# xiph/daala

Measured on NVIDIA H100. Metric: encoder Mpixels/s on 4K YUV420 intra, higher is better.
Workload: dtype int32

## Files before the change

daala_b200/csrc/kf_engine.cu:

```cuda
#include <cuda_runtime.h>
#include <math.h>
#include <stdint.h>
#include <stdio.h>
#include <stdlib.h>
#include <string.h>

#include <algorithm>
#include <cmath>
#include <mutex>
#include <new>
#include <vector>

#include "daala_b200.h"
#include "dering_search.h"
#include "late_skip.h"
#include "lossless.h"
#include "mc_batch.h"
#include "gen/coding_order.inc"
#include "pvq_math.cuh"
#include "pvq_warp.cuh"
#include "pvq_common.cuh"

namespace daala_b200 {
namespace kf {
// ... 628 lines not shown
  int top = -1, left = -1;
  if (band == 0 || r == 1) top = S.dep_top[blk];
  if (band == 0 || r == 2) left = S.dep_left[blk];
  if (band == 3 || band == 6) top = left = -1;
  const int32_t* ot = top >= 0 ? prm.out + prm.blocks[top].coef_off : nullptr;
  const int32_t* ol = left >= 0 ? prm.out + prm.blocks[left].coef_off : nullptr;
  bool low_from_top = false;
  if (band == 0) {
    double g1 = 0, g2 = 0;
    if (ot) { double a = __ldcg(ot + 2), bb = __ldcg(ot + 5), c = __ldcg(ot + 9); g1 += a * a; g1 += bb * bb; g1 += c * c; }
    if (ol) { double a = __ldcg(ol + 1), bb = __ldcg(ol + 4), c = __ldcg(ol + 7); g2 += a * a; g2 += bb * bb; g2 += c * c; }
    low_from_top = g1 > g2;
  }
  int32_t* vref = prm.ref + coef_off;
  for (int i = start + lane; i < start + bn; i += 32) {
    int r2, c2;
    scan_rc(i, &r2, &c2);
    int32_t p = 0;
    if (r2 == 0 && c2 > 0 && ot && (c2 >= 4 || low_from_top)) p = __ldcg(ot + i);
    if (c2 == 0 && r2 > 0 && ol && (r2 >= 4 || !low_from_top)) p = __ldcg(ol + i);
    vref[i] = p;
  }
}

template <bool kIntra>
__device__ __forceinline__ void run_item(const Stage& S, uint32_t item, int lane, int16_t* snap) {
  const daala_b200_pvq_params& prm = S.prm;
  const int blk = (int)(item >> 4), band = (int)(item & 15);
  const daala_b200_pvq_block b = prm.blocks[blk];
  const int bs = b.bs, pli = b.pli;
  const int start = band_start(band);
  const int bn = band_start(band + 1) - start;
  const size_t off = (size_t)b.coef_off + start;
  if (kIntra) intra_band_ref(S, blk, band, b.coef_off, lane);
  int qidx = bs * (bs + 1) + (band + 1) - (band + 1) / 3;
  int q = (prm.q0 * prm.pvq_qm_q4[pli][qidx]) >> 4;
  if (q < 1) q = 1;
  const int beta = (prm.use_masking && pli == 0 && bs > 0) ? kBeta15 : kBeta1;
  const int qoff = (b.xdec & 1 ? prm.qm_stride : 0) + ((((1 << (2 * bs)) - 1) << 4) / 3) + start;
  int itheta, max_theta, k;
  double skip_term;
  const bool pre = kIntra && S.pre_ev && band != 3 && band != 6;
  const int32_t* pev = pre ? S.pre_ev + (off >> 3) * kPreEvWords : nullptr;
  const int16_t* psn = pre ? S.pre_snap + 2 * off : nullptr;
  const int gain = quantise_band_warp<0>(lane, snap, S.rsqrt_tbl, prm.out + off, prm.in + off, prm.ref + off, bn, q,
                                         prm.y + off, &itheta, &max_theta, &k, beta, &skip_term, prm.is_keyframe, pli,
                                         prm.qm + qoff, prm.qm_inv + qoff, prm.pvq_norm_lambda, pev, psn);
  if (lane == 0) {
    const size_t r = (size_t)blk * 9 + band;
    prm.res_skip_term[r] = skip_term;
    short4 pk;
    pk.x = (short)gain; pk.y = (short)itheta; pk.z = (short)max_theta; pk.w = (short)k;
    reinterpret_cast<short4*>(S.res_pack)[r] = pk;
  }
}

struct ItemGeom {
  int blk, band, bn, q, beta, pli, qoff;
  size_t off;
};
__device__ __forceinline__ int band_q(const daala_b200_pvq_params& prm, const daala_b200_kf_frame_quant* fq, int frame,
                                      int pli, int qidx) {
  return fq ? (fq[frame].q0 * fq[frame].pvq_qm_q4[pli][qidx]) >> 4 : (prm.q0 * prm.pvq_qm_q4[pli][qidx]) >> 4;
}
__device__ __forceinline__ ItemGeom item_geom(const daala_b200_pvq_params& prm, uint32_t item,
                                              const daala_b200_kf_frame_quant* fq) {
  ItemGeom g;
  g.blk = (int)(item >> 4);
  g.band = (int)(item & 15);
  const daala_b200_pvq_block b = prm.blocks[g.blk];
  const int bs = b.bs;
  g.pli = b.pli;
  const int start = band_start(g.band);
  g.bn = band_start(g.band + 1) - start;
  g.off = (size_t)b.coef_off + start;
  const int qidx = bs * (bs + 1) + (g.band + 1) - (g.band + 1) / 3;
  int q = band_q(prm, fq, b.frame, g.pli, qidx);
  g.q = q < 1 ? 1 : q;
  g.beta = (prm.use_masking && g.pli == 0 && bs > 0) ? kBeta15 : kBeta1;
  g.qoff = (b.xdec & 1 ? prm.qm_stride : 0) + ((((1 << (2 * bs)) - 1) << 4) / 3) + start;
  return g;
}

template <int kPhase, bool kZeroRef, int kMode, bool kFq = false>
__global__ void __launch_bounds__(128) k_pvq_split(const __grid_constant__ Stage S, int cls, int chunk) {
  const daala_b200_pvq_params& prm = S.prm;
  const int lane = threadIdx.x & 31;
  const int slots = S.sp_slots[cls];
  const int first = chunk * slots;
  const int count = min(S.cnt[S.n_items_at + cls] - first, slots);
  const int vs = cls == 2 ? 128 : 32;
  const int nwarps = (gridDim.x * blockDim.x) >> 5;
  for (int i = (blockIdx.x * blockDim.x + threadIdx.x) >> 5; i < count; i += nwarps) {
    const ItemGeom g = item_geom(prm, S.items[cls][first + i], kFq ? S.fq : nullptr);
    int16_t* vec = S.sp_vec[cls] + (size_t)i * 3 * vs;
    int32_t* lanes = S.sp_lanes[cls] + (size_t)i * kCtxLaneWords * 16;
    int32_t* uni = S.sp_uni[cls] + (size_t)i * kCtxUniWords;
    int16_t* snap = S.sp_snap[cls] + (size_t)i * kMaxEvents * vs;
    const int32_t* r0 = kZeroRef ? nullptr : prm.ref + g.off;
    BandCtx B;
    if (kPhase == 0) {
      band_setup<kMode>(lane, B, prm.in + g.off, r0, g.bn, g.q, g.beta, prm.is_keyframe, g.pli, prm.qm + g.qoff,
                 prm.pvq_norm_lambda, S.rsqrt_tbl);
      band_ctx_store_setup(lane, B, g.bn, vec, vs, lanes, uni);
    } else if (kPhase == 1) {
      band_ctx_load_search(lane, B, g.bn, vec, vs, lanes);
      band_search<kMode>(lane, B, g.bn, snap, vs, S.rsqrt_tbl);
      band_ctx_store_search(lane, B, lanes);
    } else {
      band_ctx_load_finish(lane, B, g.bn, vec, vs, lanes, uni);
      int itheta, max_theta, k;
      double skip_term;
      const int gain = band_finish<kMode>(lane, B, snap, vs, prm.out + g.off, r0, g.bn, g.q, prm.y + g.off, &itheta, &max_theta, &k,
                                   g.beta, &skip_term, prm.is_keyframe, g.pli, prm.qm_inv + g.qoff, prm.pvq_norm_lambda);
      if (lane == 0) {
        const size_t r = (size_t)g.blk * 9 + g.band;
        prm.res_skip_term[r] = skip_term;
        short4 pk;
        pk.x = (short)gain; pk.y = (short)itheta; pk.z = (short)max_theta; pk.w = (short)k;
        reinterpret_cast<short4*>(S.res_pack)[r] = pk;
      }
    }
  }
}

template <int kMode>
__global__ void __launch_bounds__(128) k_pvq_prepass(const __grid_constant__ Stage S) {
  const daala_b200_pvq_params& prm = S.prm;
  __shared__ int16_t snap_all[4][2 * kMaxN];
  const int lane = threadIdx.x & 31;
  int16_t* snap = snap_all[threadIdx.x >> 5];
  const int nblk = min(S.cnt[S.n_blocks_at], S.max_blocks);
  const int nwarps = (gridDim.x * blockDim.x) >> 5;
  const int per = kMode == 2 ? 2 : 5;
  for (long long i = (blockIdx.x * blockDim.x + threadIdx.x) >> 5; i < (long long)nblk * per; i += nwarps) {
    const int blk = (int)(i / per), sel = (int)(i % per);
    const int band = kMode == 2 ? 7 + sel : (sel < 3 ? sel : sel + 1);
    if (band >= num_bands(prm.blocks[blk].bs)) continue;
    const ItemGeom g = item_geom(prm, ((uint32_t)blk << 4) | band, nullptr);
    BandCtx B;
    band_setup<kMode>(lane, B, prm.in + g.off, nullptr, g.bn, g.q, g.beta, prm.is_keyframe, g.pli, prm.qm + g.qoff,
                      prm.pvq_norm_lambda, S.rsqrt_tbl);
    band_search<kMode>(lane, B, g.bn, snap, kMaxN, S.rsqrt_tbl);
    band_noref_export(lane, B, g.bn, snap, kMaxN, S.pre_ev + (g.off >> 3) * kPreEvWords, S.pre_snap + 2 * g.off);
  }
}

__device__ __forceinline__ void grid_barrier(int32_t* bar, int* target, int nctas) {
  __syncthreads();
  if (threadIdx.x == 0) {
    *target += nctas;
    __threadfence();
    atomicAdd(bar, 1);
    while (ld_acquire(bar) < *target) {}
  }
  __syncthreads();
}

__global__ void __launch_bounds__(128, 4) k_pvq_levels(const __grid_constant__ Stage S) {
  const daala_b200_pvq_params& prm = S.prm;
  __shared__ int bar_target;
  if (threadIdx.x == 0) bar_target = 0;
  const int lane = threadIdx.x & 31;
  const int w = (blockIdx.x * blockDim.x + threadIdx.x) >> 5;
  const int nwarps = (gridDim.x * blockDim.x) >> 5;
  const int total = S.cnt[kTotalHi];
  constexpr int vs = 128;
  for (int lvl = 0; lvl < S.nlevels; lvl++) {
    const int base = S.lvl_off[lvl * 3];
    const int end = lvl + 1 < kMaxLevels ? S.lvl_off[(lvl + 1) * 3] : total;
    if (end - base > S.lvl_slots && threadIdx.x == 0 && blockIdx.x == 0) S.cnt[kError] = 2;
    const int n = min(end - base, S.lvl_slots);
    if (n <= 0) continue;
    for (int phase = 0; phase < 3; phase++) {
      for (int i = w; i < n; i += nwarps) {
        const uint32_t item = S.lvl_items[base + i];
        const ItemGeom g = item_geom(prm, item, nullptr);
        int16_t* vec = S.lv_vec + (size_t)i * 3 * vs;
        int32_t* lanes = S.lv_lanes + (size_t)i * kCtxLaneWords * 16;
        int32_t* uni = S.lv_uni + (size_t)i * kCtxUniWords;
        int16_t* snap = S.lv_snap + (size_t)i * kMaxEvents * vs;
        BandCtx B;
        if (phase == 0) {
          intra_band_ref(S, g.blk, g.band, (int)(g.off - band_start(g.band)), lane);
          band_setup<0>(lane, B, prm.in + g.off, prm.ref + g.off, g.bn, g.q, g.beta, prm.is_keyframe, g.pli,
                        prm.qm + g.qoff, prm.pvq_norm_lambda, S.rsqrt_tbl);
          band_ctx_store_setup(lane, B, g.bn, vec, vs, lanes, uni);
        } else if (phase == 1) {
          band_ctx_load_search(lane, B, g.bn, vec, vs, lanes);
          band_search<0>(lane, B, g.bn, snap, vs, S.rsqrt_tbl);
          band_ctx_store_search(lane, B, lanes);
        } else {
          band_ctx_load_finish(lane, B, g.bn, vec, vs, lanes, uni);
          int itheta, max_theta, k;
          double skip_term;
          const int gain = band_finish<0>(lane, B, snap, vs, prm.out + g.off, prm.ref + g.off, g.bn, g.q, prm.y + g.off,
                                          &itheta, &max_theta, &k, g.beta, &skip_term, prm.is_keyframe, g.pli,
                                          prm.qm_inv + g.qoff, prm.pvq_norm_lambda);
          if (lane == 0) {
            const size_t r = (size_t)g.blk * 9 + g.band;
            prm.res_skip_term[r] = skip_term;
            short4 pk;
            pk.x = (short)gain; pk.y = (short)itheta; pk.z = (short)max_theta; pk.w = (short)k;
            reinterpret_cast<short4*>(S.res_pack)[r] = pk;
// ... 507 lines not shown
  }
}

constexpr int kSymSegs = 6;
struct SymCopy {
  const uint8_t* src[kSymSegs];
  uint8_t* dst[kSymSegs];
  long long unit[kSymSegs];
  long long cap[kSymSegs];
  long long index_bytes;
  const long long* tot;
};

__global__ void __launch_bounds__(256) k_sym_copy(const __grid_constant__ SymCopy C) {
  const long long tid = (long long)blockIdx.x * blockDim.x + threadIdx.x;
  const long long nth = (long long)gridDim.x * blockDim.x;
  for (int seg = 0; seg < kSymSegs; seg++) {
    if (!C.dst[seg]) continue;
    const long long want = seg == 0 ? C.index_bytes : C.tot[seg >= 4 ? 0 : seg - 1] * C.unit[seg];
    const long long len = want < C.cap[seg] ? want : C.cap[seg];
    const uint8_t* s = C.src[seg];
    uint8_t* d = C.dst[seg];
    long long done = 0;
    if ((((uintptr_t)s | (uintptr_t)d) & 15) == 0) {
      const long long n16 = len >> 4;
      for (long long i = tid; i < n16; i += nth)
        reinterpret_cast<uint4*>(d)[i] = reinterpret_cast<const uint4*>(s)[i];
      done = n16 << 4;
    }
    for (long long i = done + tid; i < len; i += nth) d[i] = s[i];
  }
}

struct Unstream {
  const uint32_t* order;
  const long long* tot;
  const uint8_t* skip;
  const int32_t* dc;
  uint8_t* fin_skip[2];
  int32_t* fin_dc[2];
  const int32_t* form;
};

__global__ void __launch_bounds__(256) k_fin_unstream(const __grid_constant__ Unstream U) {
  if (!*U.form) return;
  const long long n = U.tot[0];
  for (long long slot = (long long)blockIdx.x * blockDim.x + threadIdx.x; slot < n;
       slot += (long long)gridDim.x * blockDim.x) {
    const uint32_t id = U.order[slot];
    const int ch = id >> 31, blk = (int)(id & 0x7fffffffu);
    U.fin_skip[ch][blk] = U.skip[slot];
    U.fin_dc[ch][blk] = U.dc[slot];
  }
}

}
}

using namespace daala_b200::kf;

extern "C" int daala_b200_launch_forward(const daala_b200_frame* prm, int nplanes, cudaStream_t stream);
extern "C" int daala_b200_launch_inverse(const daala_b200_frame* prm, int nplanes, cudaStream_t stream);
extern "C" int daala_b200_launch_inverse_lapped_only(const daala_b200_frame* prm, int plane0, int nplanes,
                                                     cudaStream_t stream);
extern "C" int daala_b200_launch_sb_postfilter_store(const daala_b200_frame* prm, int plane0, int nplanes,
                                                     cudaStream_t stream);

struct Dering {
  daala_b200_frame frame;
  const uint8_t* skip[3];
  long long skip_pitch[3];
  int skip_stride;
  uint8_t* level;
  const uint8_t* coded;
  uint8_t* applied;
  int tbl[2][6];
  const int32_t* frame_tbl;
  int32_t* thr[2];
  int32_t* dir;
  bool search;
  daala_b200_dering_search_batch sb;
};

enum { kEvLists, kEvForward, kEvLumaBands, kEvLumaScatter, kEvChroma, kNumEvents };

struct daala_b200_kf {
  daala_b200_kf_config cfg;
  int nhsb, nvsb, F;
  int plane_w[3], plane_h[3];
  cudaStream_t stream;
  bool own_stream;
  cudaStream_t side;
  cudaEvent_t ev[kNumEvents];
  cudaGraph_t graph;
  cudaGraphExec_t exec;
  bool captured;
  uint8_t* pixels[3];
  int32_t* coeffs[3];
  int32_t* lapped[3];
  uint8_t* pixels_out[3];
  uint8_t* pred_pixels[3];
  int32_t* pred_coeffs[3];
  uint8_t* bsize;
  int16_t *qm, *qm_inv;
  double* rsqrt_tbl;
  int16_t* sp_vec[3];
  int32_t* sp_lanes[3];
  int32_t* sp_uni[3];
  int16_t* sp_snap[3];
  int sp_slots[3];
  int16_t* lv_vec;
  int32_t* lv_lanes;
  int32_t* lv_uni;
  int16_t* lv_snap;
  int32_t* lv_bar;
  int lvl_slots, lvl_grid;
  Dering dering;
  Lists lists;
  Stage luma, chroma;
  Sym sym;
  daala_b200_frame frame;
  daala_b200_frame frame_pred;
  uint8_t* ref_pixels[3];
  int32_t* ref_slot;
  daala_b200_mv_pt* mv_grid;
  int32_t* ref_slot_next;
  int32_t* mv1_grid;
  uint32_t* mc_leaves;
  int32_t* mc_nleaves;
  daala_b200_mc_batch mc;
  uint8_t* fin_skip[2];
  int32_t* fin_dc[2];
  int32_t* dc_resid[2];
  int32_t* fin_coeffs[3];
  uint8_t* fin_pixels[3];
  uint8_t* fin_bskip[3];
  uint8_t *fin_level, *fin_coded;
  Fin fin;
  cudaGraph_t fin_graph;
  cudaGraphExec_t fin_exec;
  bool fin_captured;
  int fin_dc_limit;
  daala_b200_kf_frame_quant* fq;
  int32_t* fq_tbl;
  std::vector<int32_t> fq_tbl_host;
  int32_t* fin_slot_out;
  PoolStore store;
  uint8_t* fin_stream_skip;
  int32_t* fin_stream_dc;
  int32_t* fin_form;
  Unstream unstream;
  int32_t* d_orig[3];
  daala_b200_kf_late_skip* late_skip[2];
  daala_b200_late_skip_batch lsb;
  int16_t* ll_coeffs[3];
  int32_t* ll_blocks;
  int32_t* ll_dc;
  int32_t* ll_slot_out;
  daala_b200_lossless_batch ll;
  std::vector<uint8_t> slot_filled;
  bool have_step;
  daala_b200_kf_totals last_tot;
  std::vector<void*> allocs;
  size_t bytes_allocated;
  size_t chain_cap;
  int sms;
  char err[256];
// ... 535 lines not shown
      b.nhsb = kf->nhsb;
      b.nvsb = kf->nvsb;
      memcpy(b.threshold, D.tbl[0], sizeof(b.threshold));
      b.coded_quantizer = kf->cfg.coded_quantizer;
      b.qm_is_flat = kf->cfg.qm_is_flat;
      b.use_activity_masking = kf->cfg.use_masking;
      b.dering_lambda = kf->cfg.dering_lambda;
      b.bskip = D.skip[0];
      b.skip_stride = D.skip_stride;
      b.skip_pitch = D.skip_pitch[0];
      b.coded = D.coded;
      b.is_keyframe = inter ? 0 : 1;
      KF_CHECK(dalloc(kf, &b.filt, (size_t)kf->plane_w[0] * kf->plane_h[0] * F));
      KF_CHECK(dalloc(kf, &b.orig, nsb * 4096));
      KF_CHECK(dalloc(kf, &b.cand, nsb * 4096));
      KF_CHECK(dalloc(kf, &b.dist, nsb * 6));
      b.dir = D.dir;
      b.levels = D.level;
      if (kf->cfg.frame_quant) {
        b.fq = kf->fq;
        b.frame_tbl = kf->fq_tbl;
        KF_CHECK(dalloc(kf, &b.cand_thr, nsb * 5));
      }
    }
  }
  KF_CHECK(cudaDeviceSynchronize());
  k_fill_rsqrt<<<(kTableDoubles + 255) / 256, 256, 0, kf->stream>>>(kf->rsqrt_tbl);
  KF_CHECK(cudaGetLastError());
  KF_CHECK(cudaStreamSynchronize(kf->stream));
  return 0;
}

static int enqueue_recon(const daala_b200_frame& frame, int p0, int n, cudaStream_t s) {
  const int rc = daala_b200_launch_inverse_lapped_only(&frame, p0, n, s);
  return rc ? rc : daala_b200_launch_sb_postfilter_store(&frame, p0, n, s);
}

static int enqueue_dering_plane(daala_b200_kf* kf, const Dering& D, int p, cudaStream_t s) {
  const int nsb = kf->nhsb * kf->nvsb;
  const long long per = (long long)kf->plane_w[p] * kf->plane_h[p];
  daala_b200_dering_params dp;
  memset(&dp, 0, sizeof(dp));
  dp.y = nullptr;
  dp.x = D.frame.post16[p];
  dp.dir = D.dir;
  dp.bskip = D.skip[p];
  dp.sb_threshold = D.thr[p ? 1 : 0];
  dp.ystride = dp.xstride = kf->plane_w[p];
  dp.dir_stride = kf->nhsb * 8;
  dp.skip_stride = D.skip_stride;
  dp.nhsb = kf->nhsb;
  dp.nvsb = kf->nvsb;
  dp.xdec = p ? 1 : 0;
  dp.pli = p;
  dp.overlap = 1;
  dp.coeff_shift = 4;
  dp.dir_format = D.search ? 2 : 0;
  return daala_b200_dering_plane_frames(&dp, kf->F, per, per, (long long)nsb * 64, nsb, D.skip_pitch[p],
                                        D.frame.plane[p].pixels_out, s);
}

static int enqueue_dering_luma(daala_b200_kf* kf, const Dering& D, cudaStream_t s) {
  if (D.search) {
    const int rc = daala_b200_dering_search_enqueue(&D.sb, s);
    if (rc) return rc;
  }
  const int nsb = kf->nhsb * kf->nvsb;
  k_dering_thresholds<<<(kf->F * nsb + 255) / 256, 256, 0, s>>>(
      D.level, D.thr[0], D.thr[1], kf->F * nsb, make_int4(D.tbl[0][0], D.tbl[0][1], D.tbl[0][2], D.tbl[0][3]),
      make_int2(D.tbl[0][4], D.tbl[0][5]), make_int4(D.tbl[1][0], D.tbl[1][1], D.tbl[1][2], D.tbl[1][3]),
      make_int2(D.tbl[1][4], D.tbl[1][5]), D.coded, D.applied, D.frame_tbl, nsb);
  return enqueue_dering_plane(kf, D, 0, s);
}

static int enqueue_dering(daala_b200_kf* kf, const Dering& D, cudaStream_t s) {
  int rc = enqueue_recon(D.frame, 0, 3, s);
  if (!rc) rc = enqueue_dering_luma(kf, D, s);
  for (int p = 1; !rc && p < 3; p++) rc = enqueue_dering_plane(kf, D, p, s);
  return rc;
}

static int dering_launches(const Dering& D, int parts) { return 2 * parts + (D.search ? 5 + 6 + 6 + 1 : 0) + 1 + 3; }

template <bool kZeroRef, bool kFq = false>
static void enqueue_split(daala_b200_kf* kf, const Stage& S, cudaStream_t s) {
  const int grid = kf->sms * 16;
  for (int cls = 2; cls >= 0; cls--) {
    for (int chunk = 0; chunk < S.sp_chunks[cls]; chunk++) {
      if (cls == 2) {
        k_pvq_split<0, kZeroRef, 2, kFq><<<grid, 128, 0, s>>>(S, cls, chunk);
        k_pvq_split<1, kZeroRef, 2><<<grid, 128, 0, s>>>(S, cls, chunk);
        k_pvq_split<2, kZeroRef, 2, kFq><<<grid, 128, 0, s>>>(S, cls, chunk);
      } else {
        k_pvq_split<0, kZeroRef, 1, kFq><<<grid, 128, 0, s>>>(S, cls, chunk);
        k_pvq_split<1, kZeroRef, 1><<<grid, 128, 0, s>>>(S, cls, chunk);
        k_pvq_split<2, kZeroRef, 1, kFq><<<grid, 128, 0, s>>>(S, cls, chunk);
      }
    }
  }
}

template <bool kInter>
static void enqueue_sym(const Sym& Y, int wide, cudaStream_t s) {
  k_sym_rank<<<(Y.F * Y.nsb + 7) / 8, 256, 0, s>>>(Y);
  k_sym_sb_scan<<<1, 1024, 0, s>>>(Y);
  k_sym_place<<<wide, 256, 0, s>>>(Y);
  k_sym_tile_sums<<<Y.ntiles, kTile, 0, s>>>(Y);
  k_sym_tile_scan<<<1, 1024, 0, s>>>(Y);
  k_sym_offsets<<<Y.ntiles, kTile, 0, s>>>(Y);
  k_sym_pack<kInter><<<wide, 256, 0, s>>>(Y);
  k_sym_index<<<1, 256, 0, s>>>(Y);
}

static int kf_enqueue_step_inter(daala_b200_kf* kf, int phases) {
  cudaStream_t s = kf->stream;
  const Lists& L = kf->lists;
  const int wide = kf->sms * 8;
  if (phases & DAALA_B200_KF_LISTS) {
    k_unit_tile_sums<<<L.ntiles, kTile, 0, s>>>(L);
    k_tile_scan<<<1, 1024, 0, s>>>(L);
    k_unit_emit<<<L.ntiles, kTile, 0, s>>>(L);
    k_luma_items<<<wide, 256, 0, s>>>(L);
    k_chroma_items<<<wide, 256, 0, s>>>(L);
    if (kf->cfg.inter_mc) {
      if (cudaMemsetAsync(L.cnt + kMcBadRef, 0, 2 * sizeof(int32_t), s) != cudaSuccess) return (int)cudaGetLastError();
      int rc = daala_b200_launch_mc_leaves(&kf->mc, wide, s);
      if (rc) return rc;
    }
  }
  if (phases & DAALA_B200_KF_FORWARD) {
    int rc = kf->cfg.inter_mc ? daala_b200_launch_mc_obmc(&kf->mc, wide, s) : 0;
    if (!rc) rc = daala_b200_launch_forward(&kf->frame, 3, s);
    if (rc) return rc;
    for (int p = 0; kf->cfg.late_skip && p < 3; p++)
      if (cudaMemcpyAsync(kf->d_orig[p], kf->coeffs[p], sizeof(int32_t) * kf->plane_w[p] * kf->plane_h[p] * kf->F,
                          cudaMemcpyDeviceToDevice, s) != cudaSuccess)
        return (int)cudaGetLastError();
    rc = daala_b200_launch_forward(&kf->frame_pred, 3, s);
    if (rc) return rc;
  }
  const bool core = (phases & DAALA_B200_KF_SEARCH_ONLY) != 0;
  for (const Stage* S : {&kf->luma, &kf->chroma}) {
    if (!(phases & (S == &kf->luma ? DAALA_B200_KF_PVQ_LUMA : DAALA_B200_KF_PVQ_CHROMA))) continue;
    if (!core) k_gather<kGatherInter><<<wide, 256, 0, s>>>(*S);
    if (S->fq) enqueue_split<false, true>(kf, *S, s);
    else enqueue_split<false>(kf, *S, s);
    if (!core) k_finish_scatter<true><<<wide, 256, 0, s>>>(*S);
  }
  if (!core && (phases & DAALA_B200_KF_PVQ_CHROMA) && kf->cfg.late_skip) {
    const int rc = daala_b200_late_skip_enqueue(&kf->lsb, kf->sms * 3, s);
    if (rc) return rc;
  }
  if (!core && (phases & DAALA_B200_KF_PVQ_CHROMA) && kf->cfg.symbol_stream) enqueue_sym<true>(kf->sym, wide, s);
  if (phases & DAALA_B200_KF_INVERSE) {
    int rc = daala_b200_launch_inverse(&kf->frame, 3, s);
    if (rc) return rc;
  }
  return (int)cudaGetLastError();
}

static int enqueue_lists(daala_b200_kf* kf, cudaStream_t s) {
  const Lists& L = kf->lists;
  const int wide = kf->sms * 8;
  k_unit_tile_sums<<<L.ntiles, kTile, 0, s>>>(L);
  k_tile_scan<<<1, 1024, 0, s>>>(L);
  k_unit_emit<<<L.ntiles, kTile, 0, s>>>(L);
  const size_t nl = (size_t)L.max_luma * sizeof(int32_t);
  if (cudaMemsetAsync(L.succ_bottom, 0xff, nl, s) != cudaSuccess || cudaMemsetAsync(L.succ_right, 0xff, nl, s) != cudaSuccess)
    return (int)cudaGetLastError();
  if (L.lvl_hist && cudaMemsetAsync(L.lvl_hist, 0, sizeof(int32_t) * kLevelBins, s) != cudaSuccess) return (int)cudaGetLastError();
  if (cudaMemsetAsync(L.head_hist, 0, sizeof(int32_t) * kLevelBins, s) != cudaSuccess) return (int)cudaGetLastError();
  k_luma_deps<<<wide, 256, 0, s>>>(L);
  if (L.lvl_hist) {
    k_level_scan<<<1, 1024, 0, s>>>(L);
    k_level_scatter<<<wide, 256, 0, s>>>(L);
  }
  k_chroma_items<<<wide, 256, 0, s>>>(L);
  return 0;
}

static int enqueue_luma_bands(daala_b200_kf* kf, bool core, int begin, cudaStream_t s) {
  const int wide = kf->sms * 8;
  const int persist = kf->sms * (kf->cfg.persist_ctas_per_sm > 0 ? kf->cfg.persist_ctas_per_sm : kPersistCtas);
  if (cudaMemsetAsync(kf->luma.ring, 0xff, kf->chain_cap * sizeof(uint32_t), s) != cudaSuccess ||
      cudaMemsetAsync(kf->luma.join0, 0, (size_t)kf->luma.max_blocks * sizeof(int32_t), s) != cudaSuccess)
    return (int)cudaGetLastError();
  k_begin_pvq<<<1, 32, 0, s>>>(kf->lists.cnt, begin);
  if (!core) k_gather<kGatherLuma><<<wide, 256, 0, s>>>(kf->luma);
  if (kf->cfg.split_free > 1) enqueue_split<true>(kf, kf->luma, s);
  if (kf->luma.pre_ev) {
    k_pvq_prepass<2><<<kf->sms * 16, 128, 0, s>>>(kf->luma);
    k_pvq_prepass<1><<<kf->sms * 16, 128, 0, s>>>(kf->luma);
  }
  if (kf->cfg.level_chains) {
    if (cudaMemsetAsync(kf->lv_bar, 0, sizeof(int32_t) * 32, s) != cudaSuccess) return (int)cudaGetLastError();
    k_pvq_levels<<<kf->lvl_grid, 128, 0, s>>>(kf->luma);
  } else {
    k_pvq_persist<true><<<persist, kPersistThreads, 0, s>>>(kf->luma);
  }
  return 0;
}

static void enqueue_chroma(daala_b200_kf* kf, bool core, bool begin, cudaStream_t s) {
  const int wide = kf->sms * 8;
  if (begin) k_begin_pvq<<<1, 32, 0, s>>>(kf->lists.cnt, kBeginChroma);
  if (!core) k_gather<kGatherChroma><<<wide, 256, 0, s>>>(kf->chroma);
  if (kf->cfg.split_free > 0) enqueue_split<false>(kf, kf->chroma, s);
  else k_pvq_persist<false><<<kf->sms * (kf->cfg.persist_ctas_per_sm > 0 ? kf->cfg.persist_ctas_per_sm : kPersistCtas),
                              kPersistThreads, 0, s>>>(kf->chroma);
  if (!core) k_finish_scatter<false><<<wide, 256, 0, s>>>(kf->chroma);
}

static int kf_enqueue_step_forked(daala_b200_kf* kf) {
  cudaStream_t s = kf->stream, c = kf->side;
  const daala_b200_frame& fr = kf->cfg.dering ? kf->dering.frame : kf->frame;
  auto fork = [](cudaEvent_t e, cudaStream_t from, cudaStream_t to) {
    return cudaEventRecord(e, from) == cudaSuccess && cudaStreamWaitEvent(to, e, 0) == cudaSuccess;
  };
  if (!fork(kf->ev[kEvLists], s, c)) return (int)cudaGetLastError();
  int rc = daala_b200_launch_forward(&kf->frame, 3, c);
  if (!rc) rc = enqueue_lists(kf, s);
  if (rc) return rc;
  if (!fork(kf->ev[kEvForward], c, s)) return (int)cudaGetLastError();
  rc = enqueue_luma_bands(kf, false, kBeginLuma | kBeginChroma, s);
  if (rc) return rc;
  if (!fork(kf->ev[kEvLumaBands], s, c)) return (int)cudaGetLastError();
  enqueue_chroma(kf, false, false, c);
  k_finish_scatter<false><<<kf->sms * 128, 256, 0, s>>>(kf->luma);
  if (kf->cfg.symbol_stream) {
    if (!fork(kf->ev[kEvLumaScatter], s, c)) return (int)cudaGetLastError();
    enqueue_sym<false>(kf->sym, kf->sms * 8, c);
  }
  rc = enqueue_recon(fr, 1, 2, c);
  if (!rc) rc = enqueue_recon(fr, 0, 1, s);
  if (!rc && kf->cfg.dering) rc = enqueue_dering_luma(kf, kf->dering, s);
  if (rc) return rc;
  if (!fork(kf->ev[kEvChroma], c, s)) return (int)cudaGetLastError();
  for (int p = 1; kf->cfg.dering && p < 3; p++) {
    rc = enqueue_dering_plane(kf, kf->dering, p, s);
    if (rc) return rc;
  }
  return (int)cudaGetLastError();
}

static int kf_enqueue_step_lossless(daala_b200_kf* kf, int phases) {
  if (phases != DAALA_B200_KF_ALL) {
    snprintf(kf->err, sizeof(kf->err), "a lossless step runs whole (DAALA_B200_KF_ALL)");
    return (int)cudaErrorInvalidValue;
  }
  cudaStream_t s = kf->stream;
  const int wide = kf->sms * 8;
  if (kf->cfg.inter_mc) {
    if (cudaMemsetAsync(kf->lists.cnt + kMcBadRef, 0, 2 * sizeof(int32_t), s) != cudaSuccess) return (int)cudaGetLastError();
    int rc = daala_b200_launch_mc_leaves(&kf->mc, wide, s);
    if (!rc) rc = daala_b200_launch_mc_obmc(&kf->mc, wide, s);
    if (rc) return rc;
  }
  return daala_b200_launch_lossless(&kf->ll, s);
}

static int kf_enqueue_step(daala_b200_kf* kf, int phases) {
  if (kf->cfg.lossless) return kf_enqueue_step_lossless(kf, phases);
  if (kf->cfg.inter) return kf_enqueue_step_inter(kf, phases);
  if (phases == DAALA_B200_KF_ALL) return kf_enqueue_step_forked(kf);
  cudaStream_t s = kf->stream;
  if (phases & DAALA_B200_KF_LISTS) {
    const int rc = enqueue_lists(kf, s);
    if (rc) return rc;
  }
  if (phases & DAALA_B200_KF_FORWARD) {
    const int rc = daala_b200_launch_forward(&kf->frame, 3, s);
    if (rc) return rc;
  }
  const bool core = (phases & DAALA_B200_KF_SEARCH_ONLY) != 0;
  if (phases & DAALA_B200_KF_PVQ_LUMA) {
    const int rc = enqueue_luma_bands(kf, core, kBeginLuma, s);
    if (rc) return rc;
    if (!core) k_finish_scatter<false><<<kf->sms * 8, 256, 0, s>>>(kf->luma);
  }
  if (phases & DAALA_B200_KF_PVQ_CHROMA) {
    enqueue_chroma(kf, core, true, s);
    if (!core && kf->cfg.symbol_stream) enqueue_sym<false>(kf->sym, kf->sms * 8, s);
  }
  if (phases & DAALA_B200_KF_INVERSE) {
    int rc = kf->cfg.dering ? enqueue_dering(kf, kf->dering, s) : daala_b200_launch_inverse(&kf->frame, 3, s);
    if (rc) return rc;
  }
  return (int)cudaGetLastError();
}

static int kf_enqueue_finish(daala_b200_kf* kf) {
  cudaStream_t s = kf->stream;
  const int wide = kf->sms * 8;
  if (kf->fin_form) k_fin_unstream<<<wide, 256, 0, s>>>(kf->unstream);
  if (cudaMemsetAsync(kf->fin_coded, 0, (size_t)kf->F * kf->nhsb * kf->nvsb, s) != cudaSuccess)
    return (int)cudaGetLastError();
  k_fin_patch<<<wide, 256, 0, s>>>(kf->fin);
  k_fin_skip_map<<<wide, 256, 0, s>>>(kf->fin);
  const int rc = enqueue_dering(kf, kf->dering, s);
  if (rc) return rc;
  if (kf->fin_slot_out) k_fin_pool_store<<<dim3(wide > kf->F ? wide / kf->F : 1, 3 * kf->F), 256, 0, s>>>(kf->store);
  return (int)cudaGetLastError();
}

extern "C" {

static thread_local char g_create_err[256] = "null engine";

daala_b200_kf* daala_b200_kf_create(const daala_b200_kf_config* cfg) {
  snprintf(g_create_err, sizeof(g_create_err), "daala_b200_kf_create: invalid configuration");
  if (cfg && cfg->inter_mc && (cfg->inter_mc != 1 || cfg->inter != 1)) {
    snprintf(g_create_err, sizeof(g_create_err), "daala_b200_kf_create: inter_mc is 0 or 1, and 1 requires inter = 1");
    return nullptr;
  }
  if (cfg && cfg->mc_next && (cfg->mc_next != 1 || cfg->inter_mc != 1)) {
    snprintf(g_create_err, sizeof(g_create_err), "daala_b200_kf_create: mc_next is 0 or 1, and 1 requires inter_mc = 1");
    return nullptr;
  }
  if (cfg && cfg->inter_finish && (cfg->inter_finish < 0 || cfg->inter_finish > 2 || cfg->inter != 1)) {
    snprintf(g_create_err, sizeof(g_create_err),
             "daala_b200_kf_create: inter_finish is 0, 1 or 2, and 1 and 2 require inter = 1");
    return nullptr;
  }
  if (cfg && (cfg->symbol_stream < 0 || cfg->symbol_stream > 2 || (cfg->symbol_stream == 2 && cfg->inter != 1))) {
    snprintf(g_create_err, sizeof(g_create_err),
             "daala_b200_kf_create: symbol_stream is 0, 1 or 2, and 2 requires inter = 1 (a keyframe's DC goes through "
             "the Haar pyramid and has no scalar index)");
    return nullptr;
  }
  if (cfg && cfg->late_skip && (cfg->late_skip != 1 || cfg->inter != 1)) {
    snprintf(g_create_err, sizeof(g_create_err),
             "daala_b200_kf_create: late_skip is 0 or 1, and 1 requires inter = 1 (keyframes have no late skip)");
    return nullptr;
  }
  if (cfg && cfg->frame_quant && (cfg->frame_quant != 1 || cfg->inter != 1)) {
    snprintf(g_create_err, sizeof(g_create_err),
             "daala_b200_kf_create: frame_quant is 0 or 1, and 1 requires inter = 1 (a keyframe batch shares one quantizer)");
    return nullptr;
  }
  if (cfg && cfg->lossless) {
    const char* with = cfg->lossless != 1 ? "a value other than 0 or 1"
                       : cfg->dering ? "dering (lossless frames skip deringing)"
                       : cfg->symbol_stream ? "symbol_stream (the stream is the PVQ symbols)"
                       : cfg->late_skip ? "late_skip"
                       : cfg->inter_finish ? "inter_finish"
                       : cfg->frame_quant ? "frame_quant (every frame is at quantizer 0)"
                       : cfg->noref_prepass ? "noref_prepass"
                       : cfg->level_chains ? "level_chains"
                       : cfg->sb_rows > 0 ? "a row shard (sb_rows > 0)" : nullptr;
    if (with) {
      snprintf(g_create_err, sizeof(g_create_err), "daala_b200_kf_create: lossless is not defined with %s", with);
      return nullptr;
    }
  }
  if (cfg && cfg->mc_refs < 0) {
    snprintf(g_create_err, sizeof(g_create_err), "daala_b200_kf_create: mc_refs < 0");
    return nullptr;
  }
  if (cfg && cfg->inter) {
    const char* with = cfg->inter != 1 ? "a value other than 0 or 1"
                       : cfg->dering ? "dering (the all-zero skip map of the deringing stage is a keyframe property)"
                       : cfg->symbol_stream == 1 ? "symbol_stream = 1 (its block record has no DC field; "
                                                   "symbol_stream = 2 is the P-frame stream)"
                       : cfg->noref_prepass ? "noref_prepass"
// ... 21 lines not shown
    kf->cfg.sb_row0 = 0;
    kf->cfg.sb_rows = kf->nvsb;
  }
  for (int p = 0; p < 3; p++) {
    kf->plane_w[p] = (kf->nhsb * 64) >> (p ? 1 : 0);
    kf->plane_h[p] = (kf->nvsb * 64) >> (p ? 1 : 0);
  }
  if ((long long)kf->plane_w[0] * kf->plane_h[0] * kf->F >= (1ll << 31)) {
    delete kf;
    return nullptr;
  }
  int dev = 0;
  cudaDeviceProp prop;
  if (cudaGetDevice(&dev) != cudaSuccess || cudaGetDeviceProperties(&prop, dev) != cudaSuccess) {
    delete kf;
    return nullptr;
  }
  kf->sms = prop.multiProcessorCount;
  if (cfg->stream) {
    kf->stream = (cudaStream_t)cfg->stream;
  } else {
    if (cudaStreamCreateWithFlags(&kf->stream, cudaStreamNonBlocking) != cudaSuccess) {
      delete kf;
      return nullptr;
    }
    kf->own_stream = true;
  }
  if (!cfg->inter && !cfg->lossless) {
    int least = 0, greatest = 0;
    bool ok = cudaDeviceGetStreamPriorityRange(&least, &greatest) == cudaSuccess &&
              cudaStreamCreateWithPriority(&kf->side, cudaStreamNonBlocking, greatest) == cudaSuccess;
    for (int i = 0; ok && i < kNumEvents; i++) ok = cudaEventCreateWithFlags(&kf->ev[i], cudaEventDisableTiming) == cudaSuccess;
    if (!ok) {
      snprintf(g_create_err, sizeof(g_create_err), "daala_b200_kf_create: cannot create the second stream and its events");
      daala_b200_kf_destroy(kf);
      return nullptr;
    }
  }
  if (kf_alloc(kf) != 0) {
    fprintf(stderr, "daala_b200_kf_create: %s\n", kf->err);
    snprintf(g_create_err, sizeof(g_create_err), "daala_b200_kf_create: %s", kf->err);
    daala_b200_kf_destroy(kf);
    return nullptr;
  }
  return kf;
}

void daala_b200_kf_destroy(daala_b200_kf* kf) {
  if (!kf) return;
  cudaStreamSynchronize(kf->stream);
  if (kf->exec) cudaGraphExecDestroy(kf->exec);
  if (kf->graph) cudaGraphDestroy(kf->graph);
  if (kf->fin_exec) cudaGraphExecDestroy(kf->fin_exec);
  if (kf->fin_graph) cudaGraphDestroy(kf->fin_graph);
  for (void* p : kf->allocs) cudaFree(p);
  for (cudaEvent_t e : kf->ev)
    if (e) cudaEventDestroy(e);
  if (kf->side) cudaStreamDestroy(kf->side);
  if (kf->own_stream) cudaStreamDestroy(kf->stream);
  delete kf;
}

const char* daala_b200_kf_error(const daala_b200_kf* kf) { return kf ? kf->err : g_create_err; }

#ifdef DAALA_B200_CHAIN_TRACE
int daala_b200_kf_chain_trace(daala_b200_kf* kf, void** recs, int* cap) {
  if (!kf || !recs || !cap) return (int)cudaErrorInvalidValue;
  *recs = kf->luma.trace;
  *cap = kf->luma.trace_cap;
  return 0;
}
#endif

int daala_b200_kf_launches_per_step(const daala_b200_kf* kf) {
  if (!kf) return 0;
  if (kf->cfg.lossless) return (kf->cfg.inter_mc ? 2 : 0) + (kf->cfg.inter ? 1 : 2);
  auto split = [](const Stage& S) { return 3 * (S.sp_chunks[0] + S.sp_chunks[1] + S.sp_chunks[2]); };
  if (kf->cfg.inter)
    return 5 + 2 + (2 + split(kf->luma)) + (2 + split(kf->chroma)) + 2 + (kf->cfg.inter_mc ? 2 : 0) +
           (kf->cfg.symbol_stream ? 8 : 0) + (kf->cfg.late_skip ? kLateSkipLaunches : 0);
  int n = 5 + (kf->cfg.level_chains ? 2 : 0);
  n += 1;
  n += 3 + 1 + (kf->cfg.split_free > 1 ? split(kf->luma) : 0) + (kf->luma.pre_ev ? 2 : 0);
  n += 2 + (kf->cfg.split_free > 0 ? split(kf->chroma) : 1);
  n += kf->cfg.dering ? dering_launches(kf->dering, 2) : 4;
  if (kf->cfg.symbol_stream) n += 8;
  return n;
}

int daala_b200_kf_device_buffers(daala_b200_kf* kf, daala_b200_kf_buffers* out) {
  if (!kf || !out) return (int)cudaErrorInvalidValue;
  memset(out, 0, sizeof(*out));
  for (int p = 0; p < 3; p++) {
    out->pixels[p] = kf->pixels[p];
    out->coeffs[p] = kf->coeffs[p];
    out->lapped[p] = kf->lapped[p];
    out->pixels_out[p] = kf->pixels_out[p];
    out->plane_w[p] = kf->plane_w[p];
    out->plane_h[p] = kf->plane_h[p];
  }
  out->bsize = kf->bsize;
  out->counts = kf->lists.cnt;
  out->luma_blocks = kf->lists.luma;
  out->chroma_blocks = kf->lists.chroma;
  out->dep_top = kf->lists.dep_top;
  out->dep_left = kf->lists.dep_left;
  for (int c = 0; c < 3; c++) {
    out->luma_items[c] = kf->lists.items_l[c];
    out->chroma_items[c] = kf->lists.items_c[c];
  }
  out->luma_heads = kf->lists.heads;
  out->luma_heads0 = kf->lists.heads0;
  out->luma_heads_raw = kf->lists.heads_raw;
  out->luma_head_bin = kf->lists.head_bin;
  out->succ_bottom = kf->lists.succ_bottom;
  out->succ_right = kf->lists.succ_right;
  out->luma_res = kf->luma.res_pack;
  out->chroma_res = kf->chroma.res_pack;
  out->luma_y16 = kf->luma.prm.y16;
  out->chroma_y16 = kf->chroma.prm.y16;
  out->luma_skip_diff = kf->luma.prm.res_skip_diff;
  out->chroma_skip_diff = kf->chroma.prm.res_skip_diff;
  out->chroma_flip = kf->chroma.prm.res_flip;
  out->max_luma_blocks = kf->lists.max_luma;
  out->max_chroma_blocks = kf->lists.max_chroma;
  out->stream = kf->stream;
  out->bytes_allocated = (long long)kf->bytes_allocated;
  for (int p = 0; p < 3; p++) {
    out->pred_pixels[p] = kf->pred_pixels[p];
    out->pred_coeffs[p] = kf->pred_coeffs[p];
    out->ref_pixels[p] = kf->ref_pixels[p];
  }
  out->ref_slot = kf->ref_slot;
  out->mv_grid = kf->mv_grid;
  out->mc_refs = kf->cfg.mc_refs;
  out->ref_slot_next = kf->ref_slot_next;
  out->mv1_grid = kf->mv1_grid;
  out->frame_quant = kf->fq;
  return 0;
}

int daala_b200_kf_run_device(daala_b200_kf* kf, int phases, int use_graph) {
  if (!kf) return (int)cudaErrorInvalidValue;
  if (!use_graph || phases != DAALA_B200_KF_ALL) return kf_enqueue_step(kf, phases);
  if (!kf->captured) {
    int rc = kf_enqueue_step(kf, phases);
    if (rc) return rc;
    KF_CHECK(cudaStreamSynchronize(kf->stream));
    KF_CHECK(cudaStreamBeginCapture(kf->stream, cudaStreamCaptureModeThreadLocal));
    rc = kf_enqueue_step(kf, phases);
    cudaError_t e = cudaStreamEndCapture(kf->stream, &kf->graph);
    if (rc) return rc;
    KF_CHECK(e);
    KF_CHECK(cudaGraphInstantiate(&kf->exec, kf->graph, cudaGraphInstantiateFlagUseNodePriority));
    kf->captured = true;
  }
  KF_CHECK(cudaGraphLaunch(kf->exec, kf->stream));
  return 0;
}

int daala_b200_kf_time_device(daala_b200_kf* kf, int phases, int use_graph, int reps, float* ms) {
  if (!kf || !ms || reps <= 0) return (int)cudaErrorInvalidValue;
  cudaEvent_t e0, e1;
  KF_CHECK(cudaEventCreate(&e0));
  KF_CHECK(cudaEventCreate(&e1));
  if (use_graph && phases == DAALA_B200_KF_ALL && !kf->captured) {
    int rc = daala_b200_kf_run_device(kf, phases, 1);
// ... 482 lines not shown
```

Measured before the change: 2439.

## Fuse chroma CfL gather and scatter into split PVQ phase kernels

When split_free is enabled, the chroma gather and finish-scatter kernels are dropped. Their work moves into phase 0 and phase 2 of the split PVQ kernels, with per-band CfL reference flip, gather and scatter. New k_chroma_records and k_chroma_tail kernels handle per-block bookkeeping and zero the high-frequency tail. The forked schedule is reordered so the chroma tail and records overlap with luma scatter and dering. This is meant to cut separate launches and global round-trips, at the cost of more complex cross-stream ordering and a per-band flip computation that depends on when the DC band is processed.

```diff
diff --git a/daala_b200/csrc/kf_engine.cu b/daala_b200/csrc/kf_engine.cu
--- a/daala_b200/csrc/kf_engine.cu
+++ b/daala_b200/csrc/kf_engine.cu
@@ -734,8 +734,67 @@
   return g;
 }
 
-template <int kPhase, bool kZeroRef, int kMode, bool kFq = false>
-__global__ void __launch_bounds__(128) k_pvq_split(const __grid_constant__ Stage S, int cls, int chunk) {
+constexpr int kFlipScattered = 2;
+
+__device__ __forceinline__ int32_t* block_plane(const daala_b200_pvq_params& prm, const daala_b200_pvq_block& b) {
+  return prm.coef_plane[b.pli] + b.frame * prm.plane_frame_pitch[b.pli] + (size_t)b.y0 * prm.plane_stride[b.pli] + b.x0;
+}
+
+__device__ __forceinline__ void cfl_gather_band(const Stage& S, const ItemGeom& g, int lane) {
+  const daala_b200_pvq_params& prm = S.prm;
+  const daala_b200_pvq_block b = prm.blocks[g.blk];
+  const int ln = b.bs + 2;
+  const int stride = prm.plane_stride[b.pli];
+  const int32_t* src = block_plane(prm, b);
+  const int lo = S.cfl_loff[b.frame * (prm.plane_frame_pitch[b.pli] >> 4) + (long long)(b.y0 >> 2) * (stride >> 2) +
+                            (b.x0 >> 2)];
+  const int rf = g.band ? prm.res_flip[g.blk] : 0;
+  int flip;
+  if (rf & kFlipScattered) {
+    flip = rf & 1;
+  } else {
+    const int qoff = prm.qm_stride + ((((1 << (2 * b.bs)) - 1) << 4) / 3);
+    int32_t xy = 0;
+    if (lane < 15) {
+      const int i = lane + 1;
+      const int32_t rq = cfl_ref(S, b, lo, i) * prm.qm[qoff + i], inq = src[scan_to_raster(i, ln, stride)] * prm.qm[qoff + i];
+      xy = (int32_t)((rq * (int64_t)inq) >> ((kQmShift + 4) << 1));
+    }
+#pragma unroll
+    for (int o = 16; o > 0; o >>= 1) xy += __shfl_xor_sync(0xffffffffu, xy, o);
+    flip = xy < 0;
+  }
+  const int start = band_start(g.band);
+  for (int j = lane; j < g.bn; j += 32) {
+    const int32_t vr = cfl_ref(S, b, lo, start + j);
+    prm.in[g.off + j] = src[scan_to_raster(start + j, ln, stride)];
+    prm.ref[g.off + j] = flip ? -vr : vr;
+  }
+  if (g.band == 0 && lane == 0) {
+    prm.in[b.coef_off] = src[0];
+    prm.ref[b.coef_off] = cfl_ref(S, b, lo, 0);
+    prm.res_flip[g.blk] = flip;
+  }
+  __syncwarp();
+}
+
+__device__ __forceinline__ void cfl_scatter_band(const Stage& S, const ItemGeom& g, int lane) {
+  const daala_b200_pvq_params& prm = S.prm;
+  const daala_b200_pvq_block b = prm.blocks[g.blk];
+  const int ln = b.bs + 2;
+  const int stride = prm.plane_stride[b.pli];
+  int32_t* dst = block_plane(prm, b);
+  const int start = band_start(g.band);
+  __syncwarp();
+  for (int j = lane; j < g.bn; j += 32) {
+    dst[scan_to_raster(start + j, ln, stride)] = prm.out[g.off + j];
+    prm.y16[g.off + j] = (int16_t)prm.y[g.off + j];
+  }
+  if (g.band == 0 && lane == 0) prm.res_flip[g.blk] |= kFlipScattered;
+}
+
+template <int kPhase, bool kZeroRef, int kMode, bool kFq, bool kCfl>
+__device__ __forceinline__ void split_phase(const Stage& S, int cls, int chunk) {
   const daala_b200_pvq_params& prm = S.prm;
   const int lane = threadIdx.x & 31;
   const int slots = S.sp_slots[cls];
@@ -752,6 +811,7 @@
     const int32_t* r0 = kZeroRef ? nullptr : prm.ref + g.off;
     BandCtx B;
     if (kPhase == 0) {
+      if (kCfl) cfl_gather_band(S, g, lane);
       band_setup<kMode>(lane, B, prm.in + g.off, r0, g.bn, g.q, g.beta, prm.is_keyframe, g.pli, prm.qm + g.qoff,
                  prm.pvq_norm_lambda, S.rsqrt_tbl);
       band_ctx_store_setup(lane, B, g.bn, vec, vs, lanes, uni);
@@ -772,6 +832,50 @@
         pk.x = (short)gain; pk.y = (short)itheta; pk.z = (short)max_theta; pk.w = (short)k;
         reinterpret_cast<short4*>(S.res_pack)[r] = pk;
       }
+      if (kCfl) cfl_scatter_band(S, g, lane);
+    }
+  }
+}
+
+template <int kPhase, bool kZeroRef, int kMode, bool kFq = false>
+__global__ void __launch_bounds__(128) k_pvq_split(const __grid_constant__ Stage S, int cls, int chunk) {
+  split_phase<kPhase, kZeroRef, kMode, kFq, false>(S, cls, chunk);
+}
+
+template <int kPhase, int kMode>
+__global__ void __launch_bounds__(128) k_pvq_split_cfl(const __grid_constant__ Stage S, int cls, int chunk) {
+  split_phase<kPhase, false, kMode, false, true>(S, cls, chunk);
+}
+
+__global__ void __launch_bounds__(256) k_chroma_records(const __grid_constant__ Stage S) {
+  const daala_b200_pvq_params& prm = S.prm;
+  const int n = min(S.cnt[S.n_blocks_at], S.max_blocks);
+  for (int blk = blockIdx.x * blockDim.x + threadIdx.x; blk < n; blk += gridDim.x * blockDim.x) {
+    const daala_b200_pvq_block b = prm.blocks[blk];
+    const int nb = num_bands(b.bs);
+    double sd = 0;
+    for (int i = 0; i < nb; i++) sd += prm.res_skip_term[(size_t)blk * 9 + i];
+    prm.res_skip_diff[blk] = sd;
+    prm.out[b.coef_off] = prm.in[b.coef_off];
+    prm.y16[b.coef_off] = 0;
+    prm.res_flip[blk] &= 1;
+  }
+}
+
+__global__ void __launch_bounds__(256) k_chroma_tail(const __grid_constant__ Stage S) {
+  const daala_b200_pvq_params& prm = S.prm;
+  const int n = min(S.cnt[S.n_blocks_at], S.max_blocks);
+  const int lane = threadIdx.x & 31;
+  const int nwarps = (gridDim.x * blockDim.x) >> 5;
+  for (int blk = (blockIdx.x * blockDim.x + threadIdx.x) >> 5; blk < n; blk += nwarps) {
+    const daala_b200_pvq_block b = prm.blocks[blk];
+    const int ln = b.bs + 2;
+    if (ln < 5) continue;
+    const int nn = 1 << ln, stride = prm.plane_stride[b.pli];
+    int32_t* dst = block_plane(prm, b);
+    for (int i = lane; i < nn * nn; i += 32) {
+      const int r = i >> ln, c = i & (nn - 1);
+      if (!((r < 16 && c < 16) || (r < 8 && c < 32) || (c < 8 && r < 32))) dst[(size_t)r * stride + c] = 0;
     }
   }
 }
@@ -1445,7 +1549,7 @@
   daala_b200_dering_search_batch sb;
 };
 
-enum { kEvLists, kEvForward, kEvLumaBands, kEvLumaScatter, kEvChroma, kNumEvents };
+enum { kEvLists, kEvForward, kEvLumaBands, kEvChromaTail, kEvChromaBands, kEvChroma, kNumEvents };
 
 struct daala_b200_kf {
   daala_b200_kf_config cfg;
@@ -2147,19 +2251,23 @@
 
 static int dering_launches(const Dering& D, int parts) { return 2 * parts + (D.search ? 5 + 6 + 6 + 1 : 0) + 1 + 3; }
 
-template <bool kZeroRef, bool kFq = false>
+template <bool kZeroRef, bool kFq = false, bool kCfl = false>
 static void enqueue_split(daala_b200_kf* kf, const Stage& S, cudaStream_t s) {
   const int grid = kf->sms * 16;
   for (int cls = 2; cls >= 0; cls--) {
     for (int chunk = 0; chunk < S.sp_chunks[cls]; chunk++) {
       if (cls == 2) {
-        k_pvq_split<0, kZeroRef, 2, kFq><<<grid, 128, 0, s>>>(S, cls, chunk);
+        if (kCfl) k_pvq_split_cfl<0, 2><<<grid, 128, 0, s>>>(S, cls, chunk);
+        else k_pvq_split<0, kZeroRef, 2, kFq><<<grid, 128, 0, s>>>(S, cls, chunk);
         k_pvq_split<1, kZeroRef, 2><<<grid, 128, 0, s>>>(S, cls, chunk);
-        k_pvq_split<2, kZeroRef, 2, kFq><<<grid, 128, 0, s>>>(S, cls, chunk);
+        if (kCfl) k_pvq_split_cfl<2, 2><<<grid, 128, 0, s>>>(S, cls, chunk);
+        else k_pvq_split<2, kZeroRef, 2, kFq><<<grid, 128, 0, s>>>(S, cls, chunk);
       } else {
-        k_pvq_split<0, kZeroRef, 1, kFq><<<grid, 128, 0, s>>>(S, cls, chunk);
+        if (kCfl) k_pvq_split_cfl<0, 1><<<grid, 128, 0, s>>>(S, cls, chunk);
+        else k_pvq_split<0, kZeroRef, 1, kFq><<<grid, 128, 0, s>>>(S, cls, chunk);
         k_pvq_split<1, kZeroRef, 1><<<grid, 128, 0, s>>>(S, cls, chunk);
-        k_pvq_split<2, kZeroRef, 1, kFq><<<grid, 128, 0, s>>>(S, cls, chunk);
+        if (kCfl) k_pvq_split_cfl<2, 1><<<grid, 128, 0, s>>>(S, cls, chunk);
+        else k_pvq_split<2, kZeroRef, 1, kFq><<<grid, 128, 0, s>>>(S, cls, chunk);
       }
     }
   }
@@ -2269,11 +2377,23 @@
 static void enqueue_chroma(daala_b200_kf* kf, bool core, bool begin, cudaStream_t s) {
   const int wide = kf->sms * 8;
   if (begin) k_begin_pvq<<<1, 32, 0, s>>>(kf->lists.cnt, kBeginChroma);
+  if (kf->cfg.split_free > 0) {
+    if (core) enqueue_split<false>(kf, kf->chroma, s);
+    else enqueue_split<false, false, true>(kf, kf->chroma, s);
+    return;
+  }
   if (!core) k_gather<kGatherChroma><<<wide, 256, 0, s>>>(kf->chroma);
-  if (kf->cfg.split_free > 0) enqueue_split<false>(kf, kf->chroma, s);
-  else k_pvq_persist<false><<<kf->sms * (kf->cfg.persist_ctas_per_sm > 0 ? kf->cfg.persist_ctas_per_sm : kPersistCtas),
-                              kPersistThreads, 0, s>>>(kf->chroma);
+  k_pvq_persist<false><<<kf->sms * (kf->cfg.persist_ctas_per_sm > 0 ? kf->cfg.persist_ctas_per_sm : kPersistCtas),
+                         kPersistThreads, 0, s>>>(kf->chroma);
   if (!core) k_finish_scatter<false><<<wide, 256, 0, s>>>(kf->chroma);
+}
+
+static void enqueue_chroma_records(daala_b200_kf* kf, cudaStream_t s) {
+  if (kf->cfg.split_free > 0) k_chroma_records<<<kf->sms * 8, 256, 0, s>>>(kf->chroma);
+}
+
+static void enqueue_chroma_tail(daala_b200_kf* kf, cudaStream_t s) {
+  if (kf->cfg.split_free > 0) k_chroma_tail<<<kf->sms * 8, 256, 0, s>>>(kf->chroma);
 }
 
 static int kf_enqueue_step_forked(daala_b200_kf* kf) {
@@ -2291,15 +2411,18 @@
   if (rc) return rc;
   if (!fork(kf->ev[kEvLumaBands], s, c)) return (int)cudaGetLastError();
   enqueue_chroma(kf, false, false, c);
+  if (cudaEventRecord(kf->ev[kEvChromaBands], c) != cudaSuccess) return (int)cudaGetLastError();
   k_finish_scatter<false><<<kf->sms * 128, 256, 0, s>>>(kf->luma);
-  if (kf->cfg.symbol_stream) {
-    if (!fork(kf->ev[kEvLumaScatter], s, c)) return (int)cudaGetLastError();
-    enqueue_sym<false>(kf->sym, kf->sms * 8, c);
-  }
+  enqueue_chroma_tail(kf, s);
+  if (!fork(kf->ev[kEvChromaTail], s, c)) return (int)cudaGetLastError();
   rc = enqueue_recon(fr, 1, 2, c);
-  if (!rc) rc = enqueue_recon(fr, 0, 1, s);
+  if (rc) return rc;
+  rc = enqueue_recon(fr, 0, 1, s);
   if (!rc && kf->cfg.dering) rc = enqueue_dering_luma(kf, kf->dering, s);
   if (rc) return rc;
+  if (cudaStreamWaitEvent(s, kf->ev[kEvChromaBands], 0) != cudaSuccess) return (int)cudaGetLastError();
+  enqueue_chroma_records(kf, s);
+  if (kf->cfg.symbol_stream) enqueue_sym<false>(kf->sym, kf->sms * 8, s);
   if (!fork(kf->ev[kEvChroma], c, s)) return (int)cudaGetLastError();
   for (int p = 1; kf->cfg.dering && p < 3; p++) {
     rc = enqueue_dering_plane(kf, kf->dering, p, s);
@@ -2345,6 +2468,8 @@
   }
   if (phases & DAALA_B200_KF_PVQ_CHROMA) {
     enqueue_chroma(kf, core, true, s);
+    if (!core) enqueue_chroma_tail(kf, s);
+    if (!core) enqueue_chroma_records(kf, s);
     if (!core && kf->cfg.symbol_stream) enqueue_sym<false>(kf->sym, kf->sms * 8, s);
   }
   if (phases & DAALA_B200_KF_INVERSE) {
@@ -2532,7 +2657,7 @@
   int n = 5 + (kf->cfg.level_chains ? 2 : 0);
   n += 1;
   n += 3 + 1 + (kf->cfg.split_free > 1 ? split(kf->luma) : 0) + (kf->luma.pre_ev ? 2 : 0);
-  n += 2 + (kf->cfg.split_free > 0 ? split(kf->chroma) : 1);
+  n += kf->cfg.split_free > 0 ? split(kf->chroma) + 2 : 3;
   n += kf->cfg.dering ? dering_launches(kf->dering, 2) : 4;
   if (kf->cfg.symbol_stream) n += 8;
   return n;
```

Result: faster. 2464 (median of 6 runs) (+1.0%).
